# cropinghigh/sdrpp-dvbs-demodulator

Hardware: NVIDIA B200
Metric: decoded_info_gbit_s (higher is better)
Workload: dtype int8

## Files before the change

### sdrpp-dvbs-demodulator_b200/csrc/ldpc_v2.cuh

```cuda
#pragma once
#include "ldpc_decoder.cuh"
#include "ldpc_variants.h"

#include <type_traits>

namespace s2 {
namespace v2 {

constexpr int kThreads = 360;

__device__ __forceinline__ uint32_t prmt(uint32_t a, uint32_t b, uint32_t sel) {
    uint32_t d;
    asm("prmt.b32 %0, %1, %2, %3;" : "=r"(d) : "r"(a), "r"(b), "r"(sel));
    return d;
}
__device__ __forceinline__ uint32_t minu2(uint32_t a, uint32_t b) {
    uint32_t d;
    asm("min.u16x2 %0, %1, %2;" : "=r"(d) : "r"(a), "r"(b));
    return d;
}
__device__ __forceinline__ uint32_t min3u2(uint32_t a, uint32_t b, uint32_t c) {
    uint32_t d;
    asm("{.reg .b32 t; min.u16x2 t, %1, %2; min.u16x2 %0, t, %3;}" : "=r"(d) : "r"(a), "r"(b), "r"(c));
    return d;
}
__device__ __forceinline__ uint32_t addmin_relu(uint32_t a, uint32_t b, uint32_t c) {
    uint32_t d;
    asm("{.reg .b32 t; add.s16x2 t, %1, %2; min.s16x2.relu %0, t, %3;}" : "=r"(d) : "r"(a), "r"(b), "r"(c));
    return d;
}
__device__ __forceinline__ uint32_t addmin(uint32_t a, uint32_t b, uint32_t c) {
    uint32_t d;
    asm("{.reg .b32 t; add.s16x2 t, %1, %2; min.s16x2 %0, t, %3;}" : "=r"(d) : "r"(a), "r"(b), "r"(c));
    return d;
}
__device__ __forceinline__ uint32_t addmin_u32(uint32_t x, uint32_t c) {
    uint32_t d;
    asm("{.reg .b32 t; add.u32 t, %1, %2; min.u32 %0, t, %1;}" : "=r"(d) : "r"(x), "r"(c));
    return d;
}
__device__ __forceinline__ uint32_t lds_u16(uint32_t addr) {
    uint16_t v;
    asm volatile("ld.shared.u16 %0, [%1];" : "=h"(v) : "r"(addr));
    return v;
}
__device__ __forceinline__ uint32_t lds_u32(uint32_t addr) {
    uint32_t v;
    asm volatile("ld.shared.u32 %0, [%1];" : "=r"(v) : "r"(addr));
    return v;
}
__device__ __forceinline__ void sts_u16(uint32_t addr, uint32_t v) {
    asm volatile("st.shared.u16 [%0], %1;" ::"r"(addr), "h"((uint16_t)v));
}

__device__ __forceinline__ uint32_t unpack_lo(uint32_t w) { return prmt(w, 0, 0x4140); }
__device__ __forceinline__ uint32_t unpack_hi(uint32_t w) { return prmt(w, 0, 0x4342); }
__device__ __forceinline__ uint32_t pack_pair(uint32_t x) { return prmt(x, 0, 0x4420); }
__device__ __forceinline__ uint32_t pack_two(uint32_t x0, uint32_t x1) { return prmt(x0, x1, 0x6420); }
__device__ __forceinline__ uint32_t lane_mask7(uint32_t x) { return prmt(x, 0, 0xAA88); }

constexpr uint32_t kC128 = 0x00800080u, kC255 = 0x00FF00FFu, kM32 = 0xFFE0FFE0u, kP32 = 0x00200020u;
constexpr uint32_t kP63 = 0x003F003Fu, kP64 = 0x00400040u, kAllOnes = 0xFFFFFFFFu;

template <int D>
__device__ __forceinline__ void exclusive_min(const uint32_t (&a)[D], uint32_t (&ex)[D]) {
    static_assert(D >= 3, "a check has at least three links");
    uint32_t P[D], S[D + 2];
#pragma unroll
    for (int i = 1; i < D; i += 2) P[i] = (i == 1) ? minu2(a[0], a[1]) : min3u2(P[i - 2], a[i - 1], a[i]);
    constexpr int top = (D & 1) ? D - 1 : D - 2;
    S[top] = (D & 1) ? a[D - 1] : minu2(a[D - 2], a[D - 1]);
#pragma unroll
    for (int i = top - 2; i >= 0; i -= 2) S[i] = min3u2(a[i], a[i + 1], S[i + 2]);
#pragma unroll
    for (int k = 0; k < D; ++k) {
        uint32_t t[4];
        int n = 0;
        if (k & 1) {
            if (k >= 3) t[n++] = P[k - 2];
            t[n++] = a[k - 1];
        } else if (k >= 2) {
            t[n++] = P[k - 1];
        }
        if (k + 1 <= D - 1) {
            if (((k + 1) & 1) == 0 && k + 1 <= top) {
                t[n++] = S[k + 1];
            } else {
                t[n++] = a[k + 1];
                if (k + 2 <= top) t[n++] = S[k + 2];
            }
        }
        ex[k] = (n == 1) ? t[0] : (n == 2) ? minu2(t[0], t[1]) : min3u2(t[0], t[1], t[2]);
    }
}

template <int CNT, bool FIRST, bool RAGGED>
__device__ __forceinline__ void row_update(const uint32_t (&off)[CNT], int cnt, uint32_t (&mw)[(CNT + 3) / 2],
                                           uint32_t& pown, uint32_t& psec, uint32_t keep, uint32_t m1) {
    constexpr int D = CNT + 2;
    uint32_t tu[D], a[D], ex[D];
    uint32_t sx = ((D - 1) & 1) ? kC128 : 0u;
#pragma unroll
    for (int c = 0; c < D; ++c) {
        uint32_t u;
        if (c < CNT)
            u = (!RAGGED || c < cnt) ? unpack_lo(lds_u16(off[c])) : kC255;
        else
            u = (c == CNT) ? pown : psec;
        uint32_t t = u;
        if (!FIRST) {
            const uint32_t beta = (c & 1) ? unpack_hi(mw[c >> 1]) : unpack_lo(mw[c >> 1]);
            t = addmin_relu(u + beta, kM32, kC255);
        }
        tu[c] = t;
        a[c] = __vabsdiffu4(t, kC128);
        sx ^= t;
    }
    exclusive_min<D>(a, ex);
    const uint32_t ssx = lane_mask7(sx);
    uint32_t prev = 0;
#pragma unroll
    for (int c = 0; c < D; ++c) {
        const uint32_t om = addmin_relu(ex[c], kAllOnes, kP32);
        const uint32_t neg = lane_mask7(tu[c]) ^ ssx;
        const uint32_t bias = neg * 0xFFFEFFFFu + kP32;
        const uint32_t bm = addmin(om ^ neg, bias, kP63);
        const uint32_t un = addmin_relu(tu[c] + bm, kM32, kC255);
        uint32_t beta;
        asm("mad.lo.u32 %0, %1, %2, %3;" : "=r"(beta) : "r"(bm), "r"(m1), "r"(kP64));
        if (c < CNT) {
            if (!RAGGED || c < cnt) sts_u16(off[c], pack_pair(un));
        } else if (c == CNT) {
            pown = un;
        } else {
            psec = un;
        }
        if (c & 1)
            mw[c >> 1] = pack_two(prev, beta);
        else if (c == D - 1)
            mw[c >> 1] = prmt(beta, keep, 0x7620);
        prev = beta;
    }
}


__device__ __forceinline__ uint32_t win360(const uint32_t* H, int o) {
    int w = o >> 5, s = o & 31;
    uint32_t r = __funnelshift_r(__ldcg(H + w), __ldcg(H + w + 1), s);
    int over = o + 32 - 360;
    if (over > 0) r |= __ldcg(H) << (32 - over);
    return r;
}
__device__ __forceinline__ uint32_t harvest8(uint4 w, uint32_t& nzacc) {
    const uint32_t k80 = 0x80808080u;
    nzacc &= __vabsdiffu4(w.x, k80) + 0x7F7F7F7Fu;
    nzacc &= __vabsdiffu4(w.y, k80) + 0x7F7F7F7Fu;
    nzacc &= __vabsdiffu4(w.z, k80) + 0x7F7F7F7Fu;
    nzacc &= __vabsdiffu4(w.w, k80) + 0x7F7F7F7Fu;
    uint32_t a0 = prmt(w.x, w.y, 0x6420), b0 = prmt(w.x, w.y, 0x7531);
    uint32_t a1 = prmt(w.z, w.w, 0x6420), b1 = prmt(w.z, w.w, 0x7531);
    auto mask4 = [](uint32_t x) { return (((~x & 0x80808080u) >> 7) * 0x00204081u >> 21) & 0xFu; };
    return mask4(a0) | (mask4(a1) << 4) | (mask4(b0) << 8) | (mask4(b1) << 12);
}
template <bool GLOBAL, int THREADS>
__device__ __forceinline__ void harvest_planes(const uint4* src, int n360, uint32_t* H, int gstride, int tid,
                                               uint32_t& nzacc) {
    uint8_t* Hb = reinterpret_cast<uint8_t*>(H);
    for (int t = tid; t < n360 * 45; t += THREADS) {
        uint4 w = GLOBAL ? __ldcg(src + t) : src[t];
        uint32_t bits = harvest8(w, nzacc);
        int g = t / 45, k = t - g * 45;
        __stcg(&Hb[g * (kBitWords * 4) + k], (uint8_t)bits);
        __stcg(&Hb[(gstride + g) * (kBitWords * 4) + k], (uint8_t)(bits >> 8));
    }
}

template <bool STREAMED, int THREADS>
__device__ __noinline__ int full_test(const LdpcParams2& p, bool after_pass, const uint16_t* wpty, uint32_t* HP, uint32_t* HD,
                                      const uint4* vdata4, const int8_t* inA, const int8_t* inB, int* s_bad) {
    const int tid = threadIdx.x, q = p.q, K = p.K;
    uint32_t nzacc = 0xFFFFFFFFu;
    if (after_pass) {
        harvest_planes<true, THREADS>(reinterpret_cast<const uint4*>(wpty), q, HP, q, tid, nzacc);
    } else {
        const int wid = tid >> 5, lane = tid & 31;
        if (wid < 12) {
            const bool row = tid < 360;
            const unsigned wl = __activemask();
            const int8_t* ca = inA + K + (size_t)q * (row ? tid : 0);
            const int8_t* cb = inB + K + (size_t)q * (row ? tid : 0);
            for (int i = 0; i < q; ++i) {
                uint32_t w = 0x8181u;
                if (row) {
                    const uint32_t a = STREAMED ? (uint8_t)__ldcg(ca + i) : (uint8_t)__ldg(ca + i);
                    const uint32_t b = STREAMED ? (uint8_t)__ldcg(cb + i) : (uint8_t)__ldg(cb + i);
                    w = (a | (b << 8)) ^ 0x8080u;
                }
                const unsigned ba = __ballot_sync(wl, !(w & 0x80u));
                const unsigned bb = __ballot_sync(wl, !(w & 0x8000u));
                if (lane == 0) {
                    __stcg(&HP[i * kBitWords + wid], ba);
                    __stcg(&HP[(q + i) * kBitWords + wid], bb);
                }
                if ((w & 0xFFu) == 0x80u) nzacc &= ~0x00800080u;
                if ((w & 0xFF00u) == 0x8000u) nzacc &= ~0x80008000u;
            }
        }
    }
    harvest_planes<false, THREADS>(vdata4, p.ngroups, HD, p.ngroups, tid, nzacc);
    if (tid < 2) s_bad[tid] = 0;
    __syncthreads();
    if (~nzacc & 0x00800080u) atomicOr(&s_bad[0], 1);
    if (~nzacc & 0x80008000u) atomicOr(&s_bad[1], 1);
    for (int task = tid; task < q * 12; task += THREADS) {
        const int ii = task / 12, w = task - ii * 12;
        const int loff = p.layer_off[ii], cnt = (int)p.layer_off[ii + 1] - loff;
        uint32_t sA = __ldcg(&HP[ii * kBitWords + w]), sB = __ldcg(&HP[(q + ii) * kBitWords + w]);
        if (ii > 0) {
            sA ^= __ldcg(&HP[(ii - 1) * kBitWords + w]);
            sB ^= __ldcg(&HP[(q + ii - 1) * kBitWords + w]);
        } else {
            const uint32_t* ta = &HP[(q - 1) * kBitWords];
            const uint32_t* tb = &HP[(2 * q - 1) * kBitWords];
            sA ^= (__ldcg(ta + w) << 1) | (w ? __ldcg(ta + w - 1) >> 31 : 0u);
            sB ^= (__ldcg(tb + w) << 1) | (w ? __ldcg(tb + w - 1) >> 31 : 0u);
        }
        for (int c = 0; c < cnt; ++c) {
            int o = 32 * w + (int)(p.link_add[loff + c] >> 1) - 360;
            o += (o < 0) ? 360 : 0;
            const int g = p.link_group[loff + c];
            sA ^= win360(&HD[g * kBitWords], o);
            sB ^= win360(&HD[(p.ngroups + g) * kBitWords], o);
        }
        if (w == 11) {
            sA &= 0xFFu;
            sB &= 0xFFu;
        }
        if (sA) atomicOr(&s_bad[0], 1);
        if (sB) atomicOr(&s_bad[1], 1);
    }
    __syncthreads();
    return (s_bad[0] ? 1 : 0) | (s_bad[1] ? 2 : 0);
}

template <int THREADS>
__device__ __noinline__ void emit_results(const LdpcParams2& p, int fin, const int (&res)[2], int fa, int fb, bool after_pass,
                                          const uint16_t* wpty, const uint4* vdata4, const int8_t* inA, const int8_t* inB) {
    const int tid = threadIdx.x, q = p.q, K = p.K, N = p.N, R = p.R;
    const int kbytes = K / 8;
    for (int b = tid; b < kbytes; b += THREADS) {
        uint32_t nz = 0xFFFFFFFFu;
        const uint32_t bits = harvest8(vdata4[b], nz);
        if (fin & 1) p.hard_out[(size_t)fa * p.hard_stride + b] = (uint8_t)(__brev(bits & 0xFFu) >> 24);
        if (fin & 2) p.hard_out[(size_t)fb * p.hard_stride + b] = (uint8_t)(__brev((bits >> 8) & 0xFFu) >> 24);
    }
    for (int f = 0; f < 2; ++f) {
        if (!(fin >> f & 1)) continue;
        const int fr = f ? fb : fa;
        if (tid == 0) p.iters_out[fr] = (int16_t)res[f];
        if (p.llr_out) {
            int8_t* lo = p.llr_out + (size_t)fr * N;
            const uint8_t* vb = reinterpret_cast<const uint8_t*>(vdata4) + f;
            for (int x = tid; x < K; x += THREADS) lo[x] = (int8_t)(vb[2 * x] ^ 0x80u);
            if (after_pass) {
                for (int x = tid; x < R; x += THREADS) {
                    const int jj = x / q, ii = x - jj * q;
                    lo[K + x] = (int8_t)((__ldcg(&wpty[360 * ii + jj]) >> (8 * f)) ^ 0x80u);
                }
            } else {
                const int8_t* in = f ? inB : inA;
                for (int x = tid; x < R; x += THREADS) lo[K + x] = in[K + x];
            }
        }
    }
}

static __device__ __noinline__ bool wait_arrived(const unsigned int* arrived_ptr, unsigned need, long long budget) {
    const volatile unsigned* arrived = arrived_ptr;
    const long long t0 = clock64();
    while (*arrived < need) {
        __nanosleep(500);
        if (clock64() - t0 > budget) return false;
    }
    return true;
}

template <int CNT, bool RAGGED, bool STREAMED, int OCC>
__global__ void __launch_bounds__(kThreads, OCC) ldpc_v2_kernel(const __grid_constant__ LdpcParams2 p) {
    constexpr int SLOTS = CNT + 2;
    constexpr int MW = (SLOTS + 1) / 2;
    constexpr int SG = (SLOTS + 7) / 8;
    static_assert(16 * SG >= 2 * SLOTS + 2, "the message record needs two spare bytes (row level)");
    constexpr int DW = (1 + 2 * CNT + 3) & ~3;
    extern __shared__ __align__(16) uint8_t smem_raw[];
    const int q = p.q, K = p.K, N = p.N, R = p.R;
    uint16_t* vdata = reinterpret_cast<uint16_t*>(smem_raw);
    uint16_t* X = reinterpret_cast<uint16_t*>(smem_raw + (size_t)K * 2);
    uint32_t* desc = reinterpret_cast<uint32_t*>(smem_raw + (size_t)K * 2 + 768);
    __shared__ unsigned int s_pair;
    __shared__ int s_bad[2];

    const int tid = threadIdx.x;
    const int j = tid;
    const uint32_t vbase = (uint32_t)__cvta_generic_to_shared(vdata);
    uint32_t dbase = (uint32_t)__cvta_generic_to_shared(desc);
    uint32_t j2 = 2u * (uint32_t)j;
    uint32_t xaddr = (uint32_t)__cvta_generic_to_shared(X) + j2;
    uint32_t m1 = 0xFFFFFFFFu;
    uint4* wmsg = reinterpret_cast<uint4*>(p.workspace + (size_t)blockIdx.x * p.ws_stride);
    uint16_t* wpty = reinterpret_cast<uint16_t*>(p.workspace + (size_t)blockIdx.x * p.ws_stride + (size_t)q * SG * 360 * 16);
    uint32_t* HD = reinterpret_cast<uint32_t*>(reinterpret_cast<uint8_t*>(wpty) + (((size_t)R * 2 + 15) & ~(size_t)15));
    uint32_t* HP = HD + 2 * p.ngroups * kBitWords;
    {
        volatile uint4* opq = reinterpret_cast<volatile uint4*>(HP + 2 * q * kBitWords + 4) + tid;
        opq->x = j2; opq->y = xaddr; opq->z = dbase; opq->w = m1;
        j2 = opq->x; xaddr = opq->y; dbase = opq->z; m1 = opq->w;
    }
    for (int x = tid; x < q * DW; x += kThreads) {
        const int i = x / DW, w = x - i * DW;
        const int loff = p.layer_off[i], cnt = (int)p.layer_off[i + 1] - loff;
        uint32_t v = 0;
        if (w == 0) {
            v = (uint32_t)p.layer_nlev[i] | (uint32_t)p.layer_sync[i] << 8 | (uint32_t)cnt << 16;
        } else if (w <= 2 * CNT) {
            const int c = (w - 1) >> 1;
            const int k = loff + (c < cnt ? c : 0);
            v = ((w - 1) & 1) ? (uint32_t)p.link_add[k] : vbase + 720u * p.link_group[k];
        }
        desc[x] = v;
    }
    const int npairs = (p.nframes + 1) >> 1;

    for (int x = tid; x < 2 * (p.ngroups + q) * kBitWords; x += kThreads) __stcg(&HD[x], 0u);

    for (;;) {
        __syncthreads();
        if (tid == 0) {
            unsigned np = atomicAdd(p.work_counter, 1u);
            if (STREAMED && np < (unsigned)npairs) {
                if (!wait_arrived(p.arrived, min(2u * np + 2u, (unsigned)p.nframes), p.wait_budget)) np |= 0x80000000u;
                __threadfence();
            }
            s_pair = np;
        }
        __syncthreads();
        const unsigned pair_word = s_pair;
        const unsigned pair = pair_word & 0x7FFFFFFFu;
        if (pair >= (unsigned)npairs) break;
        const int fa = 2 * pair, fb = 2 * pair + 1;
        const bool hasB = fb < p.nframes;
        if (STREAMED && (pair_word & 0x80000000u)) {
            if (tid == 0) {
                p.iters_out[fa] = kLdpcItersNoInput;
                if (hasB) p.iters_out[fb] = kLdpcItersNoInput;
            }
            continue;
        }
        const int8_t* inA = p.llr_in + (size_t)fa * N;
        const int8_t* inB = p.llr_in + (size_t)(hasB ? fb : fa) * N;
        const int8_t* colA = inA + K + (size_t)q * j;
        const int8_t* colB = inB + K + (size_t)q * j;
        auto in_pair = [&](int i) -> uint32_t {
            const uint32_t a = STREAMED ? (uint8_t)__ldcg(colA + i) : (uint8_t)__ldg(colA + i);
            const uint32_t b = STREAMED ? (uint8_t)__ldcg(colB + i) : (uint8_t)__ldg(colB + i);
            return (a | (b << 8)) ^ 0x8080u;
        };

        for (int x = tid; x < K / 8; x += kThreads) {
            uint2 a = STREAMED ? __ldcg(reinterpret_cast<const uint2*>(inA) + x) : __ldg(reinterpret_cast<const uint2*>(inA) + x);
            uint2 b = STREAMED ? __ldcg(reinterpret_cast<const uint2*>(inB) + x) : __ldg(reinterpret_cast<const uint2*>(inB) + x);
            uint4 o;
            o.x = prmt(a.x, b.x, 0x5140) ^ 0x80808080u;
            o.y = prmt(a.x, b.x, 0x7362) ^ 0x80808080u;
            o.z = prmt(a.y, b.y, 0x5140) ^ 0x80808080u;
            o.w = prmt(a.y, b.y, 0x7362) ^ 0x80808080u;
            reinterpret_cast<uint4*>(vdata)[x] = o;
        }
        uint32_t pown = 0, psec = 0;
        {
            const uint32_t last = in_pair(q - 1);
            X[j + 1] = (uint16_t)last;
            pown = unpack_lo(last);
            psec = unpack_lo(in_pair(q - 2));
        }
        if (tid == 0) X[0] = 0xFFFFu;

        int live = hasB ? 3 : 1;
        uint32_t off[CNT];
        uint32_t lw0 = 0;
        auto link_addresses = [&](int i) {
            uint32_t dw[DW];
#pragma unroll
            for (int x = 0; x < DW; x += 4)
                asm volatile("ld.shared.v4.u32 {%0, %1, %2, %3}, [%4];" : "=r"(dw[x]), "=r"(dw[x + 1]), "=r"(dw[x + 2]), "=r"(dw[x + 3])
                             : "r"(dbase + (uint32_t)(i * DW + x) * 4u));
            lw0 = dw[0];
#pragma unroll
            for (int c = 0; c < CNT; ++c)
                off[c] = dw[1 + 2 * c] + addmin_u32(j2 + dw[2 + 2 * c], (uint32_t)-720);
        };
        auto screen = [&]() -> int {
            link_addresses(q - 1);
            const int cnt = (int)(lw0 >> 16);
            uint32_t sx = pown ^ psec, mn = minu2(__vabsdiffu4(pown, kC128), __vabsdiffu4(psec, kC128));
            int nl = 2;
#pragma unroll
            for (int c = 0; c < CNT; ++c) {
                if (!RAGGED || c < cnt) {
                    const uint32_t u = unpack_lo(lds_u16(off[c]));
                    sx ^= u;
                    mn = minu2(mn, __vabsdiffu4(u, kC128));
                    ++nl;
                }
            }
            if (nl & 1) sx ^= kC128;
            int bad = 0;
            if ((sx & 0x80u) || (mn & 0xFFFFu) == 0) bad |= 1;
            if ((sx & 0x800000u) || (mn >> 16) == 0) bad |= 2;
            return bad;
        };

        __syncthreads();
        int scr = screen();
        int res[2] = {-1, -1};
        for (int n = 0;; ++n) {
            int bad = (__syncthreads_or(scr & 1) ? 1 : 0) | (__syncthreads_or(scr & 2) ? 2 : 0);
            if (live & ~bad)
                bad = full_test<STREAMED, kThreads>(p, n > 0, wpty, HP, HD, reinterpret_cast<const uint4*>(vdata), inA, inB, s_bad);
            int fin = 0;
            for (int f = 0; f < 2; ++f) {
                if (!(live >> f & 1)) continue;
                if (!(bad >> f & 1)) {
                    res[f] = n;
                    fin |= 1 << f;
                } else if (n == p.max_trials) {
                    fin |= 1 << f;
                }
            }
            if (fin) {
                emit_results<kThreads>(p, fin, res, fa, fb, n > 0, wpty, reinterpret_cast<const uint4*>(vdata), inA, inB);
                live &= ~fin;
                if (live) __syncthreads();
            }
            if (!live) break;

            auto pass = [&](auto first_tag) {
                constexpr bool FIRST = decltype(first_tag)::value;
                uint32_t mw[MW];
                uint4 nxt[SG];
                uint32_t pnext = 0, pnext_b = 0;
                uint32_t pprev = 0;
#pragma unroll
                for (int x = 0; x < MW; ++x) mw[x] = 0;
                uint4* rp = wmsg + j;
                uint16_t* pp = wpty + j;
                const int8_t* ca = colA;
                const int8_t* cb = colB;
                psec = unpack_lo(lds_u16(xaddr));
                if (FIRST) {
                    pnext = STREAMED ? (uint8_t)__ldcg(ca) : (uint8_t)__ldg(ca);
                    pnext_b = STREAMED ? (uint8_t)__ldcg(cb) : (uint8_t)__ldg(cb);
                } else {
                    pnext = __ldcg(pp);
#pragma unroll
                    for (int s = 0; s < SG; ++s) nxt[s] = __ldcg(rp + s * 360);
                }
                uint32_t lev_next = (FIRST && p.layer_nlev[0] > 1) ? (uint32_t)p.row_level[j] << 24 : 0u;
                for (int i = 0; i < q; ++i) {
                    uint32_t keep = lev_next;
                    if (!FIRST) {
#pragma unroll
                        for (int s = 0; s < SG; ++s) {
                            if (4 * s + 0 < MW) mw[4 * s + 0] = nxt[s].x;
                            if (4 * s + 1 < MW) mw[4 * s + 1] = nxt[s].y;
                            if (4 * s + 2 < MW) mw[4 * s + 2] = nxt[s].z;
                            if (4 * s + 3 < MW) mw[4 * s + 3] = nxt[s].w;
                        }
                        keep = nxt[SG - 1].w;
                    }
                    const uint32_t pw = FIRST ? ((pnext | (pnext_b << 8)) ^ 0x8080u) : pnext;
                    pown = unpack_lo(i == q - 1 ? lds_u16(xaddr + 2) : pw);
                    if (i + 1 < q) {
                        if (FIRST) {
                            pnext = STREAMED ? (uint8_t)__ldcg(ca + 1) : (uint8_t)__ldg(ca + 1);
                            pnext_b = STREAMED ? (uint8_t)__ldcg(cb + 1) : (uint8_t)__ldg(cb + 1);
                        } else {
                            pnext = __ldcg(pp + 360);
#pragma unroll
                            for (int s = 0; s < SG; ++s) nxt[s] = __ldcg(rp + (SG + s) * 360);
                        }
                    }
                    link_addresses(i);
                    const int cnt = RAGGED ? (int)(lw0 >> 16) : CNT;
                    const int nlev = (int)(lw0 & 0xFFu);
                    if (FIRST) lev_next = (i + 1 < q && p.layer_nlev[i + 1] > 1) ? (uint32_t)p.row_level[(i + 1) * 360 + j] << 24 : 0u;
                    if (nlev == 1) {
                        row_update<CNT, FIRST, RAGGED>(off, cnt, mw, pown, psec, keep, m1);
                        if (lw0 & 0x100u) __syncthreads();
                    } else {
                        const int mylev = (int)(keep >> 24);
                        for (int lvl = 0; lvl < nlev; ++lvl) {
                            if (mylev == lvl) row_update<CNT, FIRST, RAGGED>(off, cnt, mw, pown, psec, keep, m1);
                            __syncthreads();
                        }
                    }
#pragma unroll
                    for (int s = 0; s < SG; ++s) {
                        uint4 o;
                        o.x = (4 * s + 0 < MW) ? mw[4 * s + 0] : 0u;
                        o.y = (4 * s + 1 < MW) ? mw[4 * s + 1] : 0u;
                        o.z = (4 * s + 2 < MW) ? mw[4 * s + 2] : 0u;
                        o.w = (4 * s + 3 < MW) ? mw[4 * s + 3] : 0u;
                        if (s == SG - 1 && 4 * s + 3 >= MW) o.w = keep & 0xFF000000u;
                        __stcg(rp + s * 360, o);
                    }
                    if (i == 0)
                        sts_u16(xaddr, pack_pair(psec));
                    else
                        __stcg(pp - 360, (uint16_t)pack_pair(psec));
                    pprev = psec;
                    psec = pown;
                    rp += SG * 360;
                    pp += 360;
                    ca += 1;
                    cb += 1;
                }
                psec = pprev;
                {
                    const uint16_t pk = (uint16_t)pack_pair(pown);
                    sts_u16(xaddr + 2, pk);
                    __stcg(pp - 360, pk);
                }
            };
            if (n == 0) pass(std::true_type{});
            else pass(std::false_type{});
            __syncthreads();
            scr = screen();
        }
    }
}

}
}

#define S2_V2_K4(c, r) {{v2::ldpc_v2_kernel<c, r, false, (c <= 9 ? 2 : 1)>, v2::ldpc_v2_kernel<c, r, false, (c <= 9 ? 3 : 2)>}, \
                        {v2::ldpc_v2_kernel<c, r, true, (c <= 9 ? 2 : 1)>, v2::ldpc_v2_kernel<c, r, true, (c <= 9 ? 3 : 2)>}}
#define S2_V2_N4 {{nullptr, nullptr}, {nullptr, nullptr}}
#define V2U(c) {c, S2_V2_K4(c, false), S2_V2_N4}
#define V2B(c) {c, S2_V2_K4(c, false), S2_V2_K4(c, true)}
#define V2R(c) {c, S2_V2_N4, S2_V2_K4(c, true)}
```

### sdrpp-dvbs-demodulator_b200/csrc/ldpc_v2l.cuh

```cuda
#pragma once
#include "ldpc_v2.cuh"

namespace s2 {
namespace v2 {

constexpr int kLdpcThreads2 = 720;

template <int NL, bool FIRST, bool RAGGED>
__device__ __forceinline__ void row_update2(const uint32_t (&off)[NL], int cntl, uint32_t (&mw)[(NL + 2) / 2], uint32_t& preg,
                                            uint32_t keep, uint32_t m1, unsigned lanes) {
    constexpr int DH = NL + 1;
    uint32_t tu[DH], a[DH];
    uint32_t sx = ((2 * DH - 1) & 1) ? kC128 : 0u;
#pragma unroll
    for (int s = 0; s < DH; ++s) {
        uint32_t u;
        if (s == 0)
            u = preg;
        else
            u = (!RAGGED || s - 1 < cntl) ? unpack_lo(lds_u16(off[s - 1])) : kC255;
        uint32_t t = u;
        if (!FIRST) {
            const uint32_t beta = (s & 1) ? unpack_hi(mw[s >> 1]) : unpack_lo(mw[s >> 1]);
            t = addmin_relu(u + beta, kM32, kC255);
        }
        tu[s] = t;
        a[s] = __vabsdiffu4(t, kC128);
        sx ^= t;
    }
    uint32_t P[DH], S[DH];
    P[0] = a[0];
#pragma unroll
    for (int s = 1; s < DH; ++s) P[s] = minu2(P[s - 1], a[s]);
    S[DH - 1] = a[DH - 1];
#pragma unroll
    for (int s = DH - 2; s >= 0; --s) S[s] = minu2(S[s + 1], a[s]);
    const uint32_t other = __shfl_xor_sync(lanes, P[DH - 1], 1);
    sx ^= __shfl_xor_sync(lanes, sx, 1) ^ (((2 * DH - 1) & 1) ? kC128 : 0u);
    const uint32_t ssx = lane_mask7(sx);
    uint32_t prev = 0;
#pragma unroll
    for (int s = 0; s < DH; ++s) {
        uint32_t ex;
        if (s == 0)
            ex = minu2(S[1], other);
        else if (s == DH - 1)
            ex = minu2(P[DH - 2], other);
        else
            ex = min3u2(P[s - 1], S[s + 1], other);
        const uint32_t om = addmin_relu(ex, kAllOnes, kP32);
        const uint32_t neg = lane_mask7(tu[s]) ^ ssx;
        const uint32_t bias = neg * 0xFFFEFFFFu + kP32;
        const uint32_t bm = addmin(om ^ neg, bias, kP63);
        const uint32_t un = addmin_relu(tu[s] + bm, kM32, kC255);
        uint32_t beta;
        asm("mad.lo.u32 %0, %1, %2, %3;" : "=r"(beta) : "r"(bm), "r"(m1), "r"(kP64));
        if (s == 0) {
            preg = un;
        } else if (!RAGGED || s - 1 < cntl) {
            sts_u16(off[s - 1], pack_pair(un));
        }
        if (s & 1)
            mw[s >> 1] = pack_two(prev, beta);
        else if (s == DH - 1)
            mw[s >> 1] = prmt(beta, keep, 0x7620);
        prev = beta;
    }
}

template <int CNT, bool RAGGED, bool STREAMED>
__global__ void __launch_bounds__(kLdpcThreads2, 1) ldpc_v2l_kernel(const __grid_constant__ LdpcParams2 p) {
    constexpr int T = kLdpcThreads2;
    constexpr int NL = (CNT + 1) / 2;
    constexpr int DH = NL + 1;
    constexpr int MW = (DH + 1) / 2;
    constexpr int SG = (DH + 7) / 8;
    static_assert(16 * SG >= 2 * DH + 2, "the message record needs two spare bytes (row level)");
    constexpr int HW = (2 * NL + 3) & ~3;
    constexpr int DW = 4 + 2 * HW;
    extern __shared__ __align__(16) uint8_t smem_raw[];
    const int q = p.q, K = p.K, N = p.N, R = p.R;
    uint16_t* vdata = reinterpret_cast<uint16_t*>(smem_raw);
    uint16_t* X = reinterpret_cast<uint16_t*>(smem_raw + (size_t)K * 2);
    uint32_t* desc = reinterpret_cast<uint32_t*>(smem_raw + (size_t)K * 2 + 768);
    __shared__ unsigned int s_pair;
    __shared__ int s_bad[2];

    const int tid = threadIdx.x;
    const int h = tid & 1;
    const int j = tid >> 1;
    const unsigned wl = __activemask();
    const int slot_t = 2 * j + h;
    const uint32_t vbase = (uint32_t)__cvta_generic_to_shared(vdata);
    uint32_t dbase = (uint32_t)__cvta_generic_to_shared(desc) + 16u + (uint32_t)h * HW * 4u;
    uint32_t j2 = 2u * (uint32_t)j;
    uint32_t xaddr = (uint32_t)__cvta_generic_to_shared(X) + j2;
    uint32_t m1 = 0xFFFFFFFFu;
    uint4* wmsg = reinterpret_cast<uint4*>(p.workspace + (size_t)blockIdx.x * p.ws_stride);
    uint16_t* wpty = reinterpret_cast<uint16_t*>(p.workspace + (size_t)blockIdx.x * p.ws_stride + (size_t)q * 2 * SG * 360 * 16);
    uint32_t* HD = reinterpret_cast<uint32_t*>(reinterpret_cast<uint8_t*>(wpty) + (((size_t)R * 2 + 15) & ~(size_t)15));
    uint32_t* HP = HD + 2 * p.ngroups * kBitWords;
    {
        volatile uint4* opq = reinterpret_cast<volatile uint4*>(HP + 2 * q * kBitWords + 4) + tid;
        opq->x = j2; opq->y = xaddr; opq->z = dbase; opq->w = m1;
        j2 = opq->x; xaddr = opq->y; dbase = opq->z; m1 = opq->w;
    }
    for (int x = tid; x < q * DW; x += T) {
        const int i = x / DW, w = x - i * DW;
        const int loff = p.layer_off[i], cnt = (int)p.layer_off[i + 1] - loff;
        uint32_t v = 0;
        if (w == 0) {
            v = (uint32_t)p.layer_nlev[i] | (uint32_t)p.layer_sync[i] << 8 | (uint32_t)cnt << 16;
        } else if (w >= 4) {
            const int hh = (w - 4) / HW, e = (w - 4) - hh * HW;
            const int s = e >> 1, d = 2 * s + hh;
            if (s < NL) {
                const int k = loff + (d < cnt ? d : 0);
                v = (e & 1) ? (uint32_t)p.link_add[k] : vbase + 720u * p.link_group[k];
            }
        }
        desc[x] = v;
    }
    const int npairs = (p.nframes + 1) >> 1;
    for (int x = tid; x < 2 * (p.ngroups + q) * kBitWords; x += T) __stcg(&HD[x], 0u);

    for (;;) {
        __syncthreads();
        if (tid == 0) {
            unsigned np = atomicAdd(p.work_counter, 1u);
            if (STREAMED && np < (unsigned)npairs) {
                if (!wait_arrived(p.arrived, min(2u * np + 2u, (unsigned)p.nframes), p.wait_budget)) np |= 0x80000000u;
                __threadfence();
            }
            s_pair = np;
        }
        __syncthreads();
        const unsigned pair_word = s_pair;
        const unsigned pair = pair_word & 0x7FFFFFFFu;
        if (pair >= (unsigned)npairs) break;
        const int fa = 2 * pair, fb = 2 * pair + 1;
        const bool hasB = fb < p.nframes;
        if (STREAMED && (pair_word & 0x80000000u)) {
            if (tid == 0) {
                p.iters_out[fa] = kLdpcItersNoInput;
                if (hasB) p.iters_out[fb] = kLdpcItersNoInput;
            }
            continue;
        }
        const int8_t* inA = p.llr_in + (size_t)fa * N;
        const int8_t* inB = p.llr_in + (size_t)(hasB ? fb : fa) * N;
        const int8_t* colA = inA + K + (size_t)q * j;
        const int8_t* colB = inB + K + (size_t)q * j;
        auto in_pair = [&](int i) -> uint32_t {
            const uint32_t a = STREAMED ? (uint8_t)__ldcg(colA + i) : (uint8_t)__ldg(colA + i);
            const uint32_t b = STREAMED ? (uint8_t)__ldcg(colB + i) : (uint8_t)__ldg(colB + i);
            return (a | (b << 8)) ^ 0x8080u;
        };

        for (int x = tid; x < K / 8; x += T) {
            uint2 a = STREAMED ? __ldcg(reinterpret_cast<const uint2*>(inA) + x) : __ldg(reinterpret_cast<const uint2*>(inA) + x);
            uint2 b = STREAMED ? __ldcg(reinterpret_cast<const uint2*>(inB) + x) : __ldg(reinterpret_cast<const uint2*>(inB) + x);
            uint4 o;
            o.x = prmt(a.x, b.x, 0x5140) ^ 0x80808080u;
            o.y = prmt(a.x, b.x, 0x7362) ^ 0x80808080u;
            o.z = prmt(a.y, b.y, 0x5140) ^ 0x80808080u;
            o.w = prmt(a.y, b.y, 0x7362) ^ 0x80808080u;
            reinterpret_cast<uint4*>(vdata)[x] = o;
        }
        uint32_t preg;
        {
            const uint32_t last = in_pair(q - 1);
            if (h == 0) X[j + 1] = (uint16_t)last;
            preg = unpack_lo(h == 0 ? last : in_pair(q - 2));
        }
        if (tid == 0) X[0] = 0xFFFFu;

        int live = hasB ? 3 : 1;
        uint32_t off[NL];
        uint32_t lw0 = 0;
        auto link_addresses = [&](int i) {
            uint32_t dw[HW];
            const uint32_t lb = dbase + (uint32_t)(i * DW) * 4u;
            lw0 = lds_u32(lb - 16u - (uint32_t)h * HW * 4u);
#pragma unroll
            for (int x = 0; x < HW; x += 4)
                asm volatile("ld.shared.v4.u32 {%0, %1, %2, %3}, [%4];" : "=r"(dw[x]), "=r"(dw[x + 1]), "=r"(dw[x + 2]), "=r"(dw[x + 3])
                             : "r"(lb + (uint32_t)x * 4u));
#pragma unroll
            for (int s = 0; s < NL; ++s) off[s] = dw[2 * s] + addmin_u32(j2 + dw[2 * s + 1], (uint32_t)-720);
        };
        auto half_links = [&](int cnt) { return (cnt - h + 1) >> 1; };
        auto screen = [&]() -> int {
            link_addresses(q - 1);
            const int cntl = half_links((int)(lw0 >> 16));
            uint32_t sx = preg, mn = __vabsdiffu4(preg, kC128);
            int nl = 1;
#pragma unroll
            for (int s = 0; s < NL; ++s) {
                if (s < cntl) {
                    const uint32_t u = unpack_lo(lds_u16(off[s]));
                    sx ^= u;
                    mn = minu2(mn, __vabsdiffu4(u, kC128));
                    ++nl;
                }
            }
            if (nl & 1) sx ^= kC128;
            sx ^= __shfl_xor_sync(wl, sx, 1);
            mn = minu2(mn, __shfl_xor_sync(wl, mn, 1));
            int bad = 0;
            if ((sx & 0x80u) || (mn & 0xFFFFu) == 0) bad |= 1;
            if ((sx & 0x800000u) || (mn >> 16) == 0) bad |= 2;
            return bad;
        };

        __syncthreads();
        int scr = screen();
        int res[2] = {-1, -1};
        for (int n = 0;; ++n) {
            int bad = (__syncthreads_or(scr & 1) ? 1 : 0) | (__syncthreads_or(scr & 2) ? 2 : 0);
            if (live & ~bad)
                bad = full_test<STREAMED, T>(p, n > 0, wpty, HP, HD, reinterpret_cast<const uint4*>(vdata), inA, inB, s_bad);
            int fin = 0;
            for (int f = 0; f < 2; ++f) {
                if (!(live >> f & 1)) continue;
                if (!(bad >> f & 1)) {
                    res[f] = n;
                    fin |= 1 << f;
                } else if (n == p.max_trials) {
                    fin |= 1 << f;
                }
            }
            if (fin) {
                emit_results<T>(p, fin, res, fa, fb, n > 0, wpty, reinterpret_cast<const uint4*>(vdata), inA, inB);
                live &= ~fin;
                if (live) __syncthreads();
            }
            if (!live) break;

            auto pass = [&](auto first_tag) {
                constexpr bool FIRST = decltype(first_tag)::value;
                uint32_t mw[MW];
                uint4 nxt[SG];
                uint32_t pnext = 0, pnext_b = 0;
#pragma unroll
                for (int x = 0; x < MW; ++x) mw[x] = 0;
                uint4* rp = wmsg + slot_t;
                uint16_t* pp = wpty + j;
                const int8_t* ca = colA;
                const int8_t* cb = colB;
                if (h == 1) preg = unpack_lo(lds_u16(xaddr));
                if (FIRST) {
                    pnext = STREAMED ? (uint8_t)__ldcg(ca) : (uint8_t)__ldg(ca);
                    pnext_b = STREAMED ? (uint8_t)__ldcg(cb) : (uint8_t)__ldg(cb);
                } else {
                    pnext = __ldcg(pp);
#pragma unroll
                    for (int s = 0; s < SG; ++s) nxt[s] = __ldcg(rp + s * 720);
                }
                uint32_t lev_next = (FIRST && p.layer_nlev[0] > 1) ? (uint32_t)p.row_level[j] << 24 : 0u;
                for (int i = 0; i < q; ++i) {
                    uint32_t keep = lev_next;
                    if (!FIRST) {
#pragma unroll
                        for (int s = 0; s < SG; ++s) {
                            if (4 * s + 0 < MW) mw[4 * s + 0] = nxt[s].x;
                            if (4 * s + 1 < MW) mw[4 * s + 1] = nxt[s].y;
                            if (4 * s + 2 < MW) mw[4 * s + 2] = nxt[s].z;
                            if (4 * s + 3 < MW) mw[4 * s + 3] = nxt[s].w;
                        }
                        keep = nxt[SG - 1].w;
                    }
                    if (h == 0) {
                        const uint32_t pw = FIRST ? ((pnext | (pnext_b << 8)) ^ 0x8080u) : pnext;
                        preg = unpack_lo(i == q - 1 ? lds_u16(xaddr + 2) : pw);
                    }
                    if (i + 1 < q) {
                        if (FIRST) {
                            pnext = STREAMED ? (uint8_t)__ldcg(ca + 1) : (uint8_t)__ldg(ca + 1);
                            pnext_b = STREAMED ? (uint8_t)__ldcg(cb + 1) : (uint8_t)__ldg(cb + 1);
                        } else {
                            pnext = __ldcg(pp + 360);
#pragma unroll
                            for (int s = 0; s < SG; ++s) nxt[s] = __ldcg(rp + (SG + s) * 720);
                        }
                    }
                    link_addresses(i);
                    const int cntl = RAGGED ? half_links((int)(lw0 >> 16)) : (h == 0 ? (CNT + 1) / 2 : CNT / 2);
                    const int nlev = (int)(lw0 & 0xFFu);
                    if (FIRST) lev_next = (i + 1 < q && p.layer_nlev[i + 1] > 1) ? (uint32_t)p.row_level[(i + 1) * 360 + j] << 24 : 0u;
                    constexpr bool kPartial = RAGGED || (CNT & 1);
                    if (nlev == 1) {
                        row_update2<NL, FIRST, kPartial>(off, cntl, mw, preg, keep, m1, wl);
                        if (lw0 & 0x100u) __syncthreads();
                    } else {
                        const int mylev = (int)(keep >> 24);
                        for (int lvl = 0; lvl < nlev; ++lvl) {
                            const unsigned lanes = __ballot_sync(wl, mylev == lvl);
                            if (mylev == lvl) row_update2<NL, FIRST, kPartial>(off, cntl, mw, preg, keep, m1, lanes);
                            __syncthreads();
                        }
                    }
#pragma unroll
                    for (int s = 0; s < SG; ++s) {
                        uint4 o;
                        o.x = (4 * s + 0 < MW) ? mw[4 * s + 0] : 0u;
                        o.y = (4 * s + 1 < MW) ? mw[4 * s + 1] : 0u;
                        o.z = (4 * s + 2 < MW) ? mw[4 * s + 2] : 0u;
                        o.w = (4 * s + 3 < MW) ? mw[4 * s + 3] : 0u;
                        if (s == SG - 1 && (4 * s + 3 >= MW || !(DH & 1))) o.w = (o.w & 0x00FFFFFFu) | (keep & 0xFF000000u);
                        __stcg(rp + s * 720, o);
                    }
                    if (h == 1) {
                        if (i == 0)
                            sts_u16(xaddr, pack_pair(preg));
                        else
                            __stcg(pp - 360, (uint16_t)pack_pair(preg));
                    }
                    const uint32_t other = __shfl_xor_sync(wl, preg, 1);
                    if (h == 1 && i + 1 < q) preg = other;
                    rp += 2 * SG * 360;
                    pp += 360;
                    ca += 1;
                    cb += 1;
                }
                if (h == 0) {
                    const uint16_t pk = (uint16_t)pack_pair(preg);
                    sts_u16(xaddr + 2, pk);
                    __stcg(pp - 360, pk);
                }
            };
            if (n == 0) pass(std::true_type{});
            else pass(std::false_type{});
            __syncthreads();
            scr = screen();
        }
    }
}

}
}

#define S2_V2L_K2(c, r) {v2::ldpc_v2l_kernel<c, r, false>, v2::ldpc_v2l_kernel<c, r, true>}
#define S2_V2L_N2 {nullptr, nullptr}
#define V2LU(c) {c, S2_V2L_K2(c, false), S2_V2L_N2}
#define V2LR(c) {c, S2_V2L_N2, S2_V2L_K2(c, true)}
```

Measured before the change: 22.21.

## Stage parity LLRs via shared-memory transpose and prefetch next frame pair into L2

Parity LLRs of both frames are now loaded with coalesced 8-byte reads, interleaved in shared memory and transposed into the global parity workspace up front. This replaces the strided per-byte column reads in the first pass, the initial syndrome test and result emission. After a frame finishes, the block also claims the next work pair early and issues a bulk L2 prefetch of its input so the next load overlaps the remaining decode. The cost is an extra staging pass with block syncs per pair and more complex work-claiming logic.

```diff
diff --git a/sdrpp-dvbs-demodulator_b200/csrc/ldpc_v2.cuh b/sdrpp-dvbs-demodulator_b200/csrc/ldpc_v2.cuh
--- a/sdrpp-dvbs-demodulator_b200/csrc/ldpc_v2.cuh
+++ b/sdrpp-dvbs-demodulator_b200/csrc/ldpc_v2.cuh
@@ -175,38 +175,12 @@
     }
 }
 
-template <bool STREAMED, int THREADS>
-__device__ __noinline__ int full_test(const LdpcParams2& p, bool after_pass, const uint16_t* wpty, uint32_t* HP, uint32_t* HD,
-                                      const uint4* vdata4, const int8_t* inA, const int8_t* inB, int* s_bad) {
-    const int tid = threadIdx.x, q = p.q, K = p.K;
+template <int THREADS>
+__device__ __noinline__ int full_test(const LdpcParams2& p, const uint16_t* wpty, uint32_t* HP, uint32_t* HD,
+                                      const uint4* vdata4, int* s_bad) {
+    const int tid = threadIdx.x, q = p.q;
     uint32_t nzacc = 0xFFFFFFFFu;
-    if (after_pass) {
-        harvest_planes<true, THREADS>(reinterpret_cast<const uint4*>(wpty), q, HP, q, tid, nzacc);
-    } else {
-        const int wid = tid >> 5, lane = tid & 31;
-        if (wid < 12) {
-            const bool row = tid < 360;
-            const unsigned wl = __activemask();
-            const int8_t* ca = inA + K + (size_t)q * (row ? tid : 0);
-            const int8_t* cb = inB + K + (size_t)q * (row ? tid : 0);
-            for (int i = 0; i < q; ++i) {
-                uint32_t w = 0x8181u;
-                if (row) {
-                    const uint32_t a = STREAMED ? (uint8_t)__ldcg(ca + i) : (uint8_t)__ldg(ca + i);
-                    const uint32_t b = STREAMED ? (uint8_t)__ldcg(cb + i) : (uint8_t)__ldg(cb + i);
-                    w = (a | (b << 8)) ^ 0x8080u;
-                }
-                const unsigned ba = __ballot_sync(wl, !(w & 0x80u));
-                const unsigned bb = __ballot_sync(wl, !(w & 0x8000u));
-                if (lane == 0) {
-                    __stcg(&HP[i * kBitWords + wid], ba);
-                    __stcg(&HP[(q + i) * kBitWords + wid], bb);
-                }
-                if ((w & 0xFFu) == 0x80u) nzacc &= ~0x00800080u;
-                if ((w & 0xFF00u) == 0x8000u) nzacc &= ~0x80008000u;
-            }
-        }
-    }
+    harvest_planes<true, THREADS>(reinterpret_cast<const uint4*>(wpty), q, HP, q, tid, nzacc);
     harvest_planes<false, THREADS>(vdata4, p.ngroups, HD, p.ngroups, tid, nzacc);
     if (tid < 2) s_bad[tid] = 0;
     __syncthreads();
@@ -244,8 +218,8 @@
 }
 
 template <int THREADS>
-__device__ __noinline__ void emit_results(const LdpcParams2& p, int fin, const int (&res)[2], int fa, int fb, bool after_pass,
-                                          const uint16_t* wpty, const uint4* vdata4, const int8_t* inA, const int8_t* inB) {
+__device__ __noinline__ void emit_results(const LdpcParams2& p, int fin, const int (&res)[2], int fa, int fb,
+                                          const uint16_t* wpty, const uint4* vdata4) {
     const int tid = threadIdx.x, q = p.q, K = p.K, N = p.N, R = p.R;
     const int kbytes = K / 8;
     for (int b = tid; b < kbytes; b += THREADS) {
@@ -262,17 +236,64 @@
             int8_t* lo = p.llr_out + (size_t)fr * N;
             const uint8_t* vb = reinterpret_cast<const uint8_t*>(vdata4) + f;
             for (int x = tid; x < K; x += THREADS) lo[x] = (int8_t)(vb[2 * x] ^ 0x80u);
-            if (after_pass) {
-                for (int x = tid; x < R; x += THREADS) {
-                    const int jj = x / q, ii = x - jj * q;
-                    lo[K + x] = (int8_t)((__ldcg(&wpty[360 * ii + jj]) >> (8 * f)) ^ 0x80u);
-                }
-            } else {
-                const int8_t* in = f ? inB : inA;
-                for (int x = tid; x < R; x += THREADS) lo[K + x] = in[K + x];
-            }
-        }
-    }
+            for (int x = tid; x < R; x += THREADS) {
+                const int jj = x / q, ii = x - jj * q;
+                lo[K + x] = (int8_t)((__ldcg(&wpty[360 * ii + jj]) >> (8 * f)) ^ 0x80u);
+            }
+        }
+    }
+}
+
+__device__ __forceinline__ uint4 interleave8(uint2 a, uint2 b) {
+    uint4 o;
+    o.x = prmt(a.x, b.x, 0x5140) ^ 0x80808080u;
+    o.y = prmt(a.x, b.x, 0x7362) ^ 0x80808080u;
+    o.z = prmt(a.y, b.y, 0x5140) ^ 0x80808080u;
+    o.w = prmt(a.y, b.y, 0x7362) ^ 0x80808080u;
+    return o;
+}
+template <bool STREAMED>
+__device__ __forceinline__ uint2 ld_in8(const int8_t* frame, int x) {
+    const uint2* s = reinterpret_cast<const uint2*>(frame) + x;
+    return STREAMED ? __ldcg(s) : __ldg(s);
+}
+
+template <bool STREAMED, int THREADS>
+__device__ __noinline__ void load_pair(const LdpcParams2& p, const int8_t* inA, const int8_t* inB, uint16_t* vdata,
+                                       uint16_t* wpty) {
+    static_assert(THREADS % 360 == 0, "a whole number of threads per column");
+    const int tid = threadIdx.x, q = p.q, K = p.K;
+    uint4* v4 = reinterpret_cast<uint4*>(vdata);
+    const int8_t* ptA = inA + K;
+    const int8_t* ptB = inB + K;
+    const int cols = min(360, (K / q) & ~7);
+    const int jj = tid % 360, i0 = tid / 360;
+    for (int j0 = 0; j0 < 360; j0 += cols) {
+        const int nc = min(cols, 360 - j0);
+        const int b8 = q * j0 / 8;
+        for (int x = tid; x < q * nc / 8; x += THREADS) v4[x] = interleave8(ld_in8<STREAMED>(ptA, b8 + x), ld_in8<STREAMED>(ptB, b8 + x));
+        __syncthreads();
+        if (jj < nc)
+            for (int i = i0; i < q; i += THREADS / 360) __stcg(&wpty[i * 360 + j0 + jj], vdata[jj * q + i]);
+        __syncthreads();
+    }
+    for (int x = tid; x < K / 8; x += THREADS) v4[x] = interleave8(ld_in8<STREAMED>(inA, x), ld_in8<STREAMED>(inB, x));
+}
+
+constexpr unsigned kNoPair = 0xFFFFFFFFu;
+template <bool STREAMED>
+__device__ __noinline__ unsigned claim_next_pair(const LdpcParams2& p, unsigned npairs) {
+    if (*reinterpret_cast<const volatile unsigned*>(p.work_counter) + gridDim.x >= npairs) return kNoPair;
+    const unsigned np = atomicAdd(p.work_counter, 1u);
+    if (np < npairs) {
+        const unsigned f0 = 2u * np, nf = min(2u, (unsigned)p.nframes - f0);
+        if (!STREAMED || *reinterpret_cast<const volatile unsigned*>(p.arrived) >= f0 + nf) {
+            const size_t b = reinterpret_cast<size_t>(p.llr_in + (size_t)f0 * p.N);
+            const size_t lo = b & ~(size_t)15, hi = (b + (size_t)nf * p.N + 15) & ~(size_t)15;
+            asm volatile("cp.async.bulk.prefetch.L2.global [%0], %1;" ::"l"(lo), "r"((unsigned)(hi - lo)) : "memory");
+        }
+    }
+    return np;
 }
 
 static __device__ __noinline__ bool wait_arrived(const unsigned int* arrived_ptr, unsigned need, long long budget) {
@@ -332,11 +353,15 @@
     const int npairs = (p.nframes + 1) >> 1;
 
     for (int x = tid; x < 2 * (p.ngroups + q) * kBitWords; x += kThreads) __stcg(&HD[x], 0u);
+    __shared__ unsigned int s_next;
+    if (tid == 0) s_next = kNoPair;
 
     for (;;) {
         __syncthreads();
         if (tid == 0) {
-            unsigned np = atomicAdd(p.work_counter, 1u);
+            unsigned np = s_next;
+            if (np == kNoPair) np = atomicAdd(p.work_counter, 1u);
+            s_next = kNoPair;
             if (STREAMED && np < (unsigned)npairs) {
                 if (!wait_arrived(p.arrived, min(2u * np + 2u, (unsigned)p.nframes), p.wait_budget)) np |= 0x80000000u;
                 __threadfence();
@@ -358,30 +383,14 @@
         }
         const int8_t* inA = p.llr_in + (size_t)fa * N;
         const int8_t* inB = p.llr_in + (size_t)(hasB ? fb : fa) * N;
-        const int8_t* colA = inA + K + (size_t)q * j;
-        const int8_t* colB = inB + K + (size_t)q * j;
-        auto in_pair = [&](int i) -> uint32_t {
-            const uint32_t a = STREAMED ? (uint8_t)__ldcg(colA + i) : (uint8_t)__ldg(colA + i);
-            const uint32_t b = STREAMED ? (uint8_t)__ldcg(colB + i) : (uint8_t)__ldg(colB + i);
-            return (a | (b << 8)) ^ 0x8080u;
-        };
-
-        for (int x = tid; x < K / 8; x += kThreads) {
-            uint2 a = STREAMED ? __ldcg(reinterpret_cast<const uint2*>(inA) + x) : __ldg(reinterpret_cast<const uint2*>(inA) + x);
-            uint2 b = STREAMED ? __ldcg(reinterpret_cast<const uint2*>(inB) + x) : __ldg(reinterpret_cast<const uint2*>(inB) + x);
-            uint4 o;
-            o.x = prmt(a.x, b.x, 0x5140) ^ 0x80808080u;
-            o.y = prmt(a.x, b.x, 0x7362) ^ 0x80808080u;
-            o.z = prmt(a.y, b.y, 0x5140) ^ 0x80808080u;
-            o.w = prmt(a.y, b.y, 0x7362) ^ 0x80808080u;
-            reinterpret_cast<uint4*>(vdata)[x] = o;
-        }
+
+        load_pair<STREAMED, kThreads>(p, inA, inB, vdata, wpty);
         uint32_t pown = 0, psec = 0;
         {
-            const uint32_t last = in_pair(q - 1);
+            const uint32_t last = __ldcg(wpty + (q - 1) * 360 + j);
             X[j + 1] = (uint16_t)last;
             pown = unpack_lo(last);
-            psec = unpack_lo(in_pair(q - 2));
+            psec = unpack_lo(__ldcg(wpty + (q - 2) * 360 + j));
         }
         if (tid == 0) X[0] = 0xFFFFu;
 
@@ -426,7 +435,7 @@
         for (int n = 0;; ++n) {
             int bad = (__syncthreads_or(scr & 1) ? 1 : 0) | (__syncthreads_or(scr & 2) ? 2 : 0);
             if (live & ~bad)
-                bad = full_test<STREAMED, kThreads>(p, n > 0, wpty, HP, HD, reinterpret_cast<const uint4*>(vdata), inA, inB, s_bad);
+                bad = full_test<kThreads>(p, wpty, HP, HD, reinterpret_cast<const uint4*>(vdata), s_bad);
             int fin = 0;
             for (int f = 0; f < 2; ++f) {
                 if (!(live >> f & 1)) continue;
@@ -438,7 +447,8 @@
                 }
             }
             if (fin) {
-                emit_results<kThreads>(p, fin, res, fa, fb, n > 0, wpty, reinterpret_cast<const uint4*>(vdata), inA, inB);
+                emit_results<kThreads>(p, fin, res, fa, fb, wpty, reinterpret_cast<const uint4*>(vdata));
+                if (tid == 0 && s_next == kNoPair) s_next = claim_next_pair<STREAMED>(p, (unsigned)npairs);
                 live &= ~fin;
                 if (live) __syncthreads();
             }
@@ -448,20 +458,15 @@
                 constexpr bool FIRST = decltype(first_tag)::value;
                 uint32_t mw[MW];
                 uint4 nxt[SG];
-                uint32_t pnext = 0, pnext_b = 0;
+                uint32_t pnext = 0;
                 uint32_t pprev = 0;
 #pragma unroll
                 for (int x = 0; x < MW; ++x) mw[x] = 0;
                 uint4* rp = wmsg + j;
                 uint16_t* pp = wpty + j;
-                const int8_t* ca = colA;
-                const int8_t* cb = colB;
                 psec = unpack_lo(lds_u16(xaddr));
-                if (FIRST) {
-                    pnext = STREAMED ? (uint8_t)__ldcg(ca) : (uint8_t)__ldg(ca);
-                    pnext_b = STREAMED ? (uint8_t)__ldcg(cb) : (uint8_t)__ldg(cb);
-                } else {
-                    pnext = __ldcg(pp);
+                pnext = __ldcg(pp);
+                if (!FIRST) {
 #pragma unroll
                     for (int s = 0; s < SG; ++s) nxt[s] = __ldcg(rp + s * 360);
                 }
@@ -478,14 +483,10 @@
                         }
                         keep = nxt[SG - 1].w;
                     }
-                    const uint32_t pw = FIRST ? ((pnext | (pnext_b << 8)) ^ 0x8080u) : pnext;
-                    pown = unpack_lo(i == q - 1 ? lds_u16(xaddr + 2) : pw);
+                    pown = unpack_lo(i == q - 1 ? lds_u16(xaddr + 2) : pnext);
                     if (i + 1 < q) {
-                        if (FIRST) {
-                            pnext = STREAMED ? (uint8_t)__ldcg(ca + 1) : (uint8_t)__ldg(ca + 1);
-                            pnext_b = STREAMED ? (uint8_t)__ldcg(cb + 1) : (uint8_t)__ldg(cb + 1);
-                        } else {
-                            pnext = __ldcg(pp + 360);
+                        pnext = __ldcg(pp + 360);
+                        if (!FIRST) {
 #pragma unroll
                             for (int s = 0; s < SG; ++s) nxt[s] = __ldcg(rp + (SG + s) * 360);
                         }
@@ -522,8 +523,6 @@
                     psec = pown;
                     rp += SG * 360;
                     pp += 360;
-                    ca += 1;
-                    cb += 1;
                 }
                 psec = pprev;
                 {
diff --git a/sdrpp-dvbs-demodulator_b200/csrc/ldpc_v2l.cuh b/sdrpp-dvbs-demodulator_b200/csrc/ldpc_v2l.cuh
--- a/sdrpp-dvbs-demodulator_b200/csrc/ldpc_v2l.cuh
+++ b/sdrpp-dvbs-demodulator_b200/csrc/ldpc_v2l.cuh
@@ -123,11 +123,15 @@
     }
     const int npairs = (p.nframes + 1) >> 1;
     for (int x = tid; x < 2 * (p.ngroups + q) * kBitWords; x += T) __stcg(&HD[x], 0u);
+    __shared__ unsigned int s_next;
+    if (tid == 0) s_next = kNoPair;
 
     for (;;) {
         __syncthreads();
         if (tid == 0) {
-            unsigned np = atomicAdd(p.work_counter, 1u);
+            unsigned np = s_next;
+            if (np == kNoPair) np = atomicAdd(p.work_counter, 1u);
+            s_next = kNoPair;
             if (STREAMED && np < (unsigned)npairs) {
                 if (!wait_arrived(p.arrived, min(2u * np + 2u, (unsigned)p.nframes), p.wait_budget)) np |= 0x80000000u;
                 __threadfence();
@@ -149,29 +153,13 @@
         }
         const int8_t* inA = p.llr_in + (size_t)fa * N;
         const int8_t* inB = p.llr_in + (size_t)(hasB ? fb : fa) * N;
-        const int8_t* colA = inA + K + (size_t)q * j;
-        const int8_t* colB = inB + K + (size_t)q * j;
-        auto in_pair = [&](int i) -> uint32_t {
-            const uint32_t a = STREAMED ? (uint8_t)__ldcg(colA + i) : (uint8_t)__ldg(colA + i);
-            const uint32_t b = STREAMED ? (uint8_t)__ldcg(colB + i) : (uint8_t)__ldg(colB + i);
-            return (a | (b << 8)) ^ 0x8080u;
-        };
-
-        for (int x = tid; x < K / 8; x += T) {
-            uint2 a = STREAMED ? __ldcg(reinterpret_cast<const uint2*>(inA) + x) : __ldg(reinterpret_cast<const uint2*>(inA) + x);
-            uint2 b = STREAMED ? __ldcg(reinterpret_cast<const uint2*>(inB) + x) : __ldg(reinterpret_cast<const uint2*>(inB) + x);
-            uint4 o;
-            o.x = prmt(a.x, b.x, 0x5140) ^ 0x80808080u;
-            o.y = prmt(a.x, b.x, 0x7362) ^ 0x80808080u;
-            o.z = prmt(a.y, b.y, 0x5140) ^ 0x80808080u;
-            o.w = prmt(a.y, b.y, 0x7362) ^ 0x80808080u;
-            reinterpret_cast<uint4*>(vdata)[x] = o;
-        }
+
+        load_pair<STREAMED, T>(p, inA, inB, vdata, wpty);
         uint32_t preg;
         {
-            const uint32_t last = in_pair(q - 1);
-            if (h == 0) X[j + 1] = (uint16_t)last;
-            preg = unpack_lo(h == 0 ? last : in_pair(q - 2));
+            const uint32_t w = __ldcg(wpty + (q - 1 - h) * 360 + j);
+            if (h == 0) X[j + 1] = (uint16_t)w;
+            preg = unpack_lo(w);
         }
         if (tid == 0) X[0] = 0xFFFFu;
 
@@ -219,7 +207,7 @@
         for (int n = 0;; ++n) {
             int bad = (__syncthreads_or(scr & 1) ? 1 : 0) | (__syncthreads_or(scr & 2) ? 2 : 0);
             if (live & ~bad)
-                bad = full_test<STREAMED, T>(p, n > 0, wpty, HP, HD, reinterpret_cast<const uint4*>(vdata), inA, inB, s_bad);
+                bad = full_test<T>(p, wpty, HP, HD, reinterpret_cast<const uint4*>(vdata), s_bad);
             int fin = 0;
             for (int f = 0; f < 2; ++f) {
                 if (!(live >> f & 1)) continue;
@@ -231,7 +219,8 @@
                 }
             }
             if (fin) {
-                emit_results<T>(p, fin, res, fa, fb, n > 0, wpty, reinterpret_cast<const uint4*>(vdata), inA, inB);
+                emit_results<T>(p, fin, res, fa, fb, wpty, reinterpret_cast<const uint4*>(vdata));
+                if (tid == 0 && s_next == kNoPair) s_next = claim_next_pair<STREAMED>(p, (unsigned)npairs);
                 live &= ~fin;
                 if (live) __syncthreads();
             }
@@ -241,19 +230,14 @@
                 constexpr bool FIRST = decltype(first_tag)::value;
                 uint32_t mw[MW];
                 uint4 nxt[SG];
-                uint32_t pnext = 0, pnext_b = 0;
+                uint32_t pnext = 0;
 #pragma unroll
                 for (int x = 0; x < MW; ++x) mw[x] = 0;
                 uint4* rp = wmsg + slot_t;
                 uint16_t* pp = wpty + j;
-                const int8_t* ca = colA;
-                const int8_t* cb = colB;
                 if (h == 1) preg = unpack_lo(lds_u16(xaddr));
-                if (FIRST) {
-                    pnext = STREAMED ? (uint8_t)__ldcg(ca) : (uint8_t)__ldg(ca);
-                    pnext_b = STREAMED ? (uint8_t)__ldcg(cb) : (uint8_t)__ldg(cb);
-                } else {
-                    pnext = __ldcg(pp);
+                pnext = __ldcg(pp);
+                if (!FIRST) {
 #pragma unroll
                     for (int s = 0; s < SG; ++s) nxt[s] = __ldcg(rp + s * 720);
                 }
@@ -270,16 +254,11 @@
                         }
                         keep = nxt[SG - 1].w;
                     }
-                    if (h == 0) {
-                        const uint32_t pw = FIRST ? ((pnext | (pnext_b << 8)) ^ 0x8080u) : pnext;
-                        preg = unpack_lo(i == q - 1 ? lds_u16(xaddr + 2) : pw);
-                    }
+                    if (h == 0)
+                        preg = unpack_lo(i == q - 1 ? lds_u16(xaddr + 2) : pnext);
                     if (i + 1 < q) {
-                        if (FIRST) {
-                            pnext = STREAMED ? (uint8_t)__ldcg(ca + 1) : (uint8_t)__ldg(ca + 1);
-                            pnext_b = STREAMED ? (uint8_t)__ldcg(cb + 1) : (uint8_t)__ldg(cb + 1);
-                        } else {
-                            pnext = __ldcg(pp + 360);
+                        pnext = __ldcg(pp + 360);
+                        if (!FIRST) {
 #pragma unroll
                             for (int s = 0; s < SG; ++s) nxt[s] = __ldcg(rp + (SG + s) * 720);
                         }
@@ -320,8 +299,6 @@
                     if (h == 1 && i + 1 < q) preg = other;
                     rp += 2 * SG * 360;
                     pp += 360;
-                    ca += 1;
-                    cb += 1;
                 }
                 if (h == 0) {
                     const uint16_t pk = (uint16_t)pack_pair(preg);
```

Result: faster. 23.69, median of 6 (+6.7%).
